# UMEssen/Body-and-Organ-Analysis

Hardware: AMD Instinct MI355X
Metric: CT volumes/sec (512^3 @1.5 mm, total+bca) on MI355X (higher is better)
Workload: dtype f16

## Files before the change

### body-and-organ-analysis_amd/csrc/conv_ns.hip

```cpp
#include <stdlib.h>

#include "conv.h"

#include "conv_ws_dev.h"

#define NS_SW_ROW 24
#define NS_SW_YODD 5
#define NS_SW_ZODD 10
__host__ __device__ constexpr int ns_sw_yp(int y) { return (y & 1) * NS_SW_YODD + (y >> 1); }
__host__ __device__ constexpr int ns_sw_zp(int z) { return (z & 1) * NS_SW_ZODD + (z >> 1); }
__host__ __device__ constexpr int ns_sw_slots() { return 9 * 9 * NS_SW_ROW; }
__host__ __device__ constexpr int ns_sw_plane_bytes() { return (ns_sw_slots() + 8) * 16 + 64; }

template <bool X3, bool SS, bool EDGE>
__device__ __forceinline__ void ns_commit_items_sw(const ConvArgs& p, const ChunkRegs& rg, unsigned char* d0, const int (&off)[WS_MAXV], int plane,
                                                   int nv, unsigned slope2) {
    if (EDGE)
        asm volatile("; commit sw: edge tile");
    else
        asm volatile("; commit sw: interior tile");
#pragma unroll
    for (int j = 0; j < WS_MAXV; ++j) {
        if (j < nv) {
            if constexpr (X3) {
                float y[4] = {__uint_as_float(rg.d[j].x), __uint_as_float(rg.d[j].y), __uint_as_float(rg.d[j].z), __uint_as_float(rg.d[j].w)};
                if (SS) {
#pragma unroll
                    for (int i = 0; i < 4; ++i) {
                        const float f = __builtin_fmaf(y[i], __uint_as_float(rg.ssw[2 * i]), __uint_as_float(rg.ssw[2 * i + 1]));
                        y[i] = f > 0.f ? f : f * p.slope;
                    }
                }
                uint2 hi, lo;
                x3_split4(y, hi, lo);
                if (EDGE && !((rg.ok >> j) & 1u)) hi = lo = make_uint2(0, 0);
                *(uint2*)(d0 + off[j]) = hi;
                *(uint2*)(d0 + plane + off[j]) = lo;
            } else {
                uint4 o = rg.d[j];
                if (SS) o = norm_act8_pk(o, rg.ssw, slope2);
                if (EDGE && !((rg.ok >> j) & 1u)) o = make_uint4(0, 0, 0, 0);
                *(uint4*)(d0 + off[j]) = o;
            }
        }
    }
}

template <bool X3>
__device__ __forceinline__ void ns_commit_sw(const ConvArgs& p, ChunkRegs& rg, unsigned char* dst_in, const int (&off)[WS_MAXV], int q, int HV,
                                             int plane, int dbg) {
    const int nv = (dbg & 32) ? 0 : (HV + WS_PROD / 2 - 1) / (WS_PROD / 2);
    if (rg.skip_halo) return;
    union {
        unsigned u;
        h2_t v;
    } sl2;
    sl2.v = h2_t{(_Float16)p.slope, (_Float16)p.slope};
    unsigned char* d0 = X3 ? dst_in + (q & 1) * 8 : dst_in + (q & 1) * plane;
    const bool edge = __builtin_amdgcn_ballot_w64(rg.ok != rg.live) != 0;
    if (rg.has_ss) {
        if (edge)
            ns_commit_items_sw<X3, true, true>(p, rg, d0, off, plane, nv, sl2.u);
        else
            ns_commit_items_sw<X3, true, false>(p, rg, d0, off, plane, nv, sl2.u);
    } else {
        if (edge)
            ns_commit_items_sw<X3, false, true>(p, rg, d0, off, plane, nv, sl2.u);
        else
            ns_commit_items_sw<X3, false, false>(p, rg, d0, off, plane, nv, sl2.u);
    }
}

template <int S, int RM, bool X3, int NR>
__device__ __forceinline__ void consume_chunk_x(const unsigned char* b0p, f32x16 (&acc)[RM], f16x8 (&a)[NR][3], f16x8 (&al)[X3 ? NR : 1][3],
                                                const WS_GLOBAL unsigned char* wb, unsigned vcur, unsigned vnext, unsigned gs, unsigned lo_off) {
    constexpr int NB = S * (RM - 1) + 3;
    constexpr int MM = X3 ? 2 : 1;
    f16x8 b[NB];
    auto fetch_a = [&](unsigned vchunk, int g, int slot) {
#pragma unroll
        for (int dx = 0; dx < 3; ++dx) {
            unsigned vo = __umul24((unsigned)(g + 9 * dx), gs) + vchunk;
            asm volatile("" : "+v"(vo));
            a[slot][dx] = *(const WS_GLOBAL f16x8*)(wb + vo);
            if constexpr (X3) {
                unsigned vl = vo + lo_off;
                asm volatile("" : "+v"(vl));
                al[slot][dx] = *(const WS_GLOBAL f16x8*)(wb + vl);
            }
        }
    };
#pragma unroll
    for (int jj = 0; jj < NB; ++jj) b[jj] = *(const f16x8*)(b0p + jj * 9 * NS_SW_ROW * 16);
    __builtin_amdgcn_sched_group_barrier(0x100, NB, 0);
#pragma unroll
    for (int g = 0; g < 9; ++g) {
        const int slot = g % NR;
        if (g + NR - 1 < 9)
            fetch_a(vcur, g + NR - 1, (g + NR - 1) % NR);
        else
            fetch_a(vnext, g + NR - 1 - 9, (g + NR - 1) % NR);
        __builtin_amdgcn_sched_group_barrier(0x020, 3 * MM, 0);
#pragma unroll
        for (int jj = 0; jj < NB; ++jj) {
            int cnt = 0;
#pragma unroll
            for (int dx = 0; dx < 3; ++dx) {
                const int rr = jj - dx;
                if (rr < 0 || rr % S != 0 || rr / S >= RM) continue;
                const int r = rr / S;
                acc[r] = __builtin_amdgcn_mfma_f32_32x32x16_f16(a[slot][dx], b[jj], acc[r], 0, 0, 0);
                if constexpr (X3) acc[r] = __builtin_amdgcn_mfma_f32_32x32x16_f16(al[slot][dx], b[jj], acc[r], 0, 0, 0);
                ++cnt;
            }
            if (cnt == 1)
                __builtin_amdgcn_sched_group_barrier(0x008, 1 * MM, 0);
            else if (cnt == 2)
                __builtin_amdgcn_sched_group_barrier(0x008, 2 * MM, 0);
            else if (cnt == 3)
                __builtin_amdgcn_sched_group_barrier(0x008, 3 * MM, 0);
            if (g + 1 < 9) {
                const int gn = g + 1, dy = gn / 3, dz = gn % 3;
                b[jj] = *(const f16x8*)(b0p + ((jj * 9 + ns_sw_yp(dy)) * NS_SW_ROW + ns_sw_zp(dz)) * 16);
                __builtin_amdgcn_sched_group_barrier(0x100, 1, 0);
            }
        }
    }
}

template <int S, int WN, int RM, bool X3>
__global__ __launch_bounds__(WS_THREADS) void k_conv_ns(ConvArgs p, int dbg_arg, const int* __restrict__ desc, int desc_row) {
    static_assert(S == 2, "k_conv_ns: the halo layout is the stride-2 one");
#ifdef WS_WITH_TRACE
    const int dbg = dbg_arg;
#else
    constexpr int dbg = 0;
    (void)dbg_arg;
#endif
    extern __shared__ __attribute__((aligned(16))) unsigned char smem[];
    const int tid = threadIdx.x;
    const int lane = tid & 63;
    const int wave = __builtin_amdgcn_readfirstlane(tid >> 6);
    const bool producer = wave >= 4;
    const int l31 = lane & 31;
    const int kh = lane >> 5;
    const int HV = p.h0 * p.h1 * p.h2;
    const int plane = ns_sw_plane_bytes();
    const int ncc = (p.C0 + p.C1) / 16;
    const int buf_bytes = 2 * plane;
    unsigned char* bufs = smem;

    const int* __restrict__ drow = desc + (size_t)blockIdx.x * desc_row * 8;
    const int my_tiles = drow[0];
    const int my_chunks = my_tiles * ncc;
    for (int i = tid; i < p.Cout; i += WS_THREADS) ((float*)(smem + 2 * buf_bytes))[i] = p.bias[i];
    const int tr_blk = WS_TRACING ? (int)p.trace[WS_TRACE_SLOTS - 5] : -1;

    if (producer) {
        const int q = tid - 256;
        const ProdConst pc = prod_const(p, q, HV);
        int ldso[WS_MAXV];
#pragma unroll
        for (int j = 0; j < WS_MAXV; ++j) {
            const int v = (q >> 1) + (WS_PROD / 2) * j;
            const int hz = v % 17, t = v / 17;
            const int hy = t % 9, hx = t / 9;
            ldso[j] = (v < HV ? (hx * 9 + ns_sw_yp(hy)) * NS_SW_ROW + ns_sw_zp(hz) : ns_sw_slots()) * 16;
        }
        TileDesc pd;
        pd.flags = pd.vo = pd.ibase = 0;
        TileCoord& ptc = pd.tc;
        int pk = 0;
        ptc.n = ptc.cy = ptc.ox0 = ptc.oy0 = ptc.oz0 = ptc.sp = 0;
        ProdItems items;
#pragma unroll
        for (int j = 0; j < WS_MAXV; ++j) items.gi[j] = 0;
        items.ok = 0;
        constexpr bool PF2 = RM == 4;
        ChunkRegs rgA, rgB;
        auto clear_regs = [&](ChunkRegs& rg) {
#pragma unroll
            for (int j = 0; j < WS_MAXV; ++j) rg.d[j] = make_uint4(0, 0, 0, 0);
#pragma unroll
            for (int j = 0; j < 8; ++j) rg.ssw[j] = 0;
            rg.ok = rg.live = 0;
            rg.has_ss = 0;
            rg.skip_halo = 0;
            rg.cc = rg.cy = 0;
        };
        clear_regs(rgA);
        clear_regs(rgB);
        int pcc = 0;
        int ptr_n = 0;
#define NS_PSTAMP(code)                                                                                                          \
    do {                                                                                                                         \
        if (WS_TRACING && (int)blockIdx.x == tr_blk && wave == 4 && lane == 0 && ptr_n < WS_TRACE_SLOTS / 2 - 8) {                                  \
            p.trace[WS_TRACE_SLOTS / 2 + ptr_n] = ((unsigned long long)(code) << 56) | (__builtin_readcyclecounter() & 0x00ffffffffffffffull); \
            ++ptr_n;                                                                                                             \
        }                                                                                                                        \
    } while (0)
        const bool live = !(dbg & 2);
        auto setup_next = [&]() {
            pd = load_desc(drow, ++pk);
            prod_setup_desc(p, pd, pc, items);
            NS_PSTAMP(8);
        };
        auto issue = [&](ChunkRegs& rg) {
            prod_issue(p, ptc, items, pc.in_halo, pcc, false, q, dbg, rg);
            if (++pcc == ncc) pcc = 0;
            NS_PSTAMP(3);
        };
        auto commit = [&](ChunkRegs& rg, unsigned char* dst) {
            if (WS_TRACING) {
                asm volatile("s_waitcnt vmcnt(0)" ::: "memory");
                NS_PSTAMP(7);
            }
            ns_commit_sw<X3>(p, rg, dst, ldso, q, HV, plane, dbg);
            NS_PSTAMP(2);
        };
        if (live && my_chunks > 0) {
            pd = load_desc(drow, 0);
            prod_setup_desc(p, pd, pc, items);
            prod_issue(p, ptc, items, pc.in_halo, 0, false, q, dbg, rgA);
            if (++pcc == ncc) pcc = 0;
        }
        if constexpr (PF2) {
            auto interval = [&](int g, ChunkRegs& cur, ChunkRegs& nxt) {
                if (live && g + 1 < my_chunks) {
                    NS_PSTAMP(1);
                    if (g + 2 < my_chunks) {
                        if (pcc == 0) setup_next();
                        issue(nxt);
                    }
                    commit(cur, bufs + ((g + 1) & 1) * buf_bytes);
                }
                __syncthreads();
            };
            for (int g = -1; g < my_chunks; g += 2) {
                interval(g, rgA, rgB);
                if (g + 1 < my_chunks) interval(g + 1, rgB, rgA);
            }
        } else {
            for (int g = -1; g < my_chunks; ++g) {
                if (live && g + 1 < my_chunks) {
                    NS_PSTAMP(1);
                    const bool do_issue = g + 2 < my_chunks;
                    if (do_issue && pcc == 0) setup_next();
                    commit(rgA, bufs + ((g + 1) & 1) * buf_bytes);
                    if (do_issue) issue(rgA);
                }
                __syncthreads();
            }
        }
        return;
    }

    if (!(dbg & 1024)) __builtin_amdgcn_s_setprio(3);
    int tr_n = 0;
#define NS_STAMP(code)                                                                                                   \
    do {                                                                                                                 \
        if (WS_TRACING && (int)blockIdx.x == tr_blk && wave == 0 && lane == 0 && tr_n < WS_TRACE_SLOTS / 2) {                              \
            p.trace[tr_n] = ((unsigned long long)(code) << 56) | (__builtin_readcyclecounter() & 0x00ffffffffffffffull); \
            ++tr_n;                                                                                                      \
        }                                                                                                                \
    } while (0)
    const int cw = wave & 3;
    const int wn = cw % WN, wm = cw / WN;
    const int ly = l31 >> 3, lz = l31 & 7;
    const int nchunks_out = p.Cout / 32;
    const int hoff = (((2 * (wm * RM)) * 9 + ly) * NS_SW_ROW + lz) * 16 + kh * plane;
    const int srel0 = ly * p.Wo + lz;
    const size_t out_vox = (size_t)p.Do * p.Ho * p.Wo;
    const int nslots = p.nslots;
    int slot = 0;
    float st_s[16], st_q[16];
#pragma unroll
    for (int i = 0; i < 16; ++i) st_s[i] = st_q[i] = 0.f;
    int st_n = -1, st_ch = 0;
    auto flush_stats = [&]() {
        if (st_n < 0) return;
#define NS_HALVE(M, HALF)                                                                                \
    {                                                                                                    \
        const bool up = (l31 & (M)) != 0;                                                                \
        _Pragma("unroll") for (int i = 0; i < (HALF); ++i) {                                             \
            const float ks = up ? st_s[i + (HALF)] : st_s[i], gs_ = up ? st_s[i] : st_s[i + (HALF)];     \
            const float kq = up ? st_q[i + (HALF)] : st_q[i], gq_ = up ? st_q[i] : st_q[i + (HALF)];     \
            st_s[i] = ks + __shfl_xor(gs_, (M));                                                         \
            st_q[i] = kq + __shfl_xor(gq_, (M));                                                         \
        }                                                                                                \
    }
        NS_HALVE(1, 8)
        NS_HALVE(2, 4)
        NS_HALVE(4, 2)
        NS_HALVE(8, 1)
#undef NS_HALVE
        st_s[0] += __shfl_xor(st_s[0], 16);
        st_q[0] += __shfl_xor(st_q[0], 16);
        if (l31 < 16) {
            const int i = ((l31 & 1) << 3) | ((l31 & 2) << 1) | ((l31 & 4) >> 1) | ((l31 & 8) >> 3);
            const int row = st_ch * 32 + 8 * (i >> 2) + 4 * kh + (i & 3);
            float* pp = p.partials + (((size_t)st_n * p.Cout + row) * 2) * nslots + slot;
            pp[0] = st_s[0];
            pp[nslots] = st_q[0];
        }
#pragma unroll
        for (int i = 0; i < 16; ++i) st_s[i] = st_q[i] = 0.f;
    };

    f32x16 acc[RM];
    auto epilogue = [&](const TileCoord& tc, int ch, int dfl, int dvo) {
        st_n = tc.n;
        st_ch = ch;
        const int cout0 = ch * 32;
        const bool full = (dfl & WS_DF_FULL) != 0;
        const size_t ovox = (size_t)(unsigned)dvo;
        const size_t obase = ((size_t)tc.n * p.Cout + cout0) * out_vox + ovox * 16;
        const unsigned olane = ((unsigned)kh * (unsigned)out_vox + (unsigned)srel0) * 32u;
#pragma unroll
        for (int r = 0; r < RM; ++r) {
            const int mx = wm * RM + r;
            const int mrel = mx * p.Ho * p.Wo;
            bool ok = true;
            if (!full) ok = tc.ox0 + mx < p.Do && tc.oy0 + ly < p.Ho && tc.oz0 + lz < p.Wo;
            const float dm = ok ? 1.f : 0.f;
            float v[16];
#pragma unroll
            for (int i = 0; i < 16; ++i) v[i] = X3 ? acc[r][i] * p.winv : acc[r][i];
#pragma unroll
            for (int i = 0; i < 8; ++i) {
                f2_t vm = f2_t{v[2 * i], v[2 * i + 1]};
                if (!full) vm = vm * f2_t{dm, dm};
                f2_t s2 = f2_t{st_s[2 * i], st_s[2 * i + 1]}, q2 = f2_t{st_q[2 * i], st_q[2 * i + 1]};
                s2 = s2 + vm;
                q2 = __builtin_elementwise_fma(vm, vm, q2);
                st_s[2 * i] = s2.x; st_s[2 * i + 1] = s2.y;
                st_q[2 * i] = q2.x; st_q[2 * i + 1] = q2.y;
            }
            if constexpr (X3) {
                if (ok && !(dbg & 4)) {
                    const size_t doff = ((size_t)tc.n * p.Cout + cout0) * out_vox * 4 + (ovox + (size_t)mrel) * 32;
                    const unsigned dlo = __builtin_amdgcn_readfirstlane((unsigned)doff), dhi = __builtin_amdgcn_readfirstlane((unsigned)(doff >> 32));
                    WS_GLOBAL unsigned char* dst = sgpr_ptr((const unsigned char*)p.out + (((size_t)dhi << 32) | dlo));
#pragma unroll
                    for (int gq = 0; gq < 4; ++gq) {
                        unsigned ol = ((unsigned)srel0 * 32u + (unsigned)kh * 16u) + (unsigned)gq * ((unsigned)out_vox * 32u);
                        asm volatile("" : "+v"(ol));
                        __builtin_nontemporal_store(f32x4_t{v[gq * 4 + 0], v[gq * 4 + 1], v[gq * 4 + 2], v[gq * 4 + 3]}, (WS_GLOBAL f32x4_t*)(dst + ol));
                    }
                }
                continue;
            }
            __builtin_amdgcn_sched_barrier(0);
            unsigned w[8];
#pragma unroll
            for (int pr = 0; pr < 2; ++pr) {
                float lo4[4], hi4[4];
#pragma unroll
                for (int e = 0; e < 4; ++e) {
                    const auto sw = __builtin_amdgcn_permlane32_swap(__float_as_uint(v[pr * 4 + e]), __float_as_uint(v[(pr + 2) * 4 + e]), false, false);
                    lo4[e] = __uint_as_float(sw[0]);
                    hi4[e] = __uint_as_float(sw[1]);
                }
                w[pr * 4 + 0] = cvt_pk_h2(lo4[0], lo4[1]);
                w[pr * 4 + 1] = cvt_pk_h2(lo4[2], lo4[3]);
                w[pr * 4 + 2] = cvt_pk_h2(hi4[0], hi4[1]);
                w[pr * 4 + 3] = cvt_pk_h2(hi4[2], hi4[3]);
            }
            if (ok && !(dbg & 4)) {
                WS_GLOBAL unsigned char* dst = sgpr_ptr(p.out + (obase + (size_t)mrel * 16));
                unsigned ol = olane;
                asm volatile("" : "+v"(ol));
                __builtin_nontemporal_store(u32x4_t{w[0], w[1], w[2], w[3]}, (WS_GLOBAL u32x4_t*)(dst + ol));
                __builtin_nontemporal_store(u32x4_t{w[4], w[5], w[6], w[7]}, (WS_GLOBAL u32x4_t*)(dst + ol + 16));
            }
        }
    };

    const unsigned gs = 32u * (unsigned)p.Cout;
    const unsigned voff = X3 ? (unsigned)l31 * 16u : ((unsigned)kh * (unsigned)p.Cout + (unsigned)l31) * 16u;
    const unsigned lo_off = (unsigned)p.Cout * 16u;
    auto woff = [&](int cc, int ch) -> unsigned { return voff + (unsigned)cc * 27u * gs + (unsigned)ch * 512u; };
    constexpr int NR = (RM == 2 && !X3) ? 9 : 3;
    f16x8 a[NR][3];
    f16x8 al[X3 ? NR : 1][3];
#pragma unroll
    for (int i = 0; i < NR; ++i)
#pragma unroll
        for (int j = 0; j < 3; ++j)
#pragma unroll
            for (int e = 0; e < 8; ++e) {
                a[i][j][e] = (_Float16)0.f;
                if (X3 || i == 0) al[X3 ? i : 0][j][e] = (_Float16)0.f;
            }
    auto prime = [&](unsigned vchunk) {
        const WS_GLOBAL unsigned char* wb = sgpr_ptr(p.wpk);
#pragma unroll
        for (int g = 0; g < NR - 1; ++g)
#pragma unroll
            for (int dx = 0; dx < 3; ++dx) {
                unsigned vo = __umul24((unsigned)(g + 9 * dx), gs) + vchunk;
                asm volatile("" : "+v"(vo));
                a[g][dx] = *(const WS_GLOBAL f16x8*)(wb + vo);
                if constexpr (X3) {
                    unsigned vl = vo + lo_off;
                    asm volatile("" : "+v"(vl));
                    al[g][dx] = *(const WS_GLOBAL f16x8*)(wb + vl);
                }
            }
    };

    TileDesc cd;
    cd.flags = cd.vo = cd.ibase = 0;
    cd.tc.n = cd.tc.cy = cd.tc.ox0 = cd.tc.oy0 = cd.tc.oz0 = cd.tc.sp = 0;
    bool ring_valid = false;
    TileCoord done_tc = cd.tc;
    int done_ch = 0, done_fl = 0, done_vo = 0;
    bool done_active = false;
    __syncthreads();
    for (int k = 0; k < my_tiles + 1; ++k) {
        const bool more = k < my_tiles;
        bool new_run = true;
        NS_STAMP(1);
        if (more) {
            cd = load_desc(drow, k);
            new_run = (cd.flags & WS_DF_NEWRUN) != 0;
        }
        const bool have_next = k + 1 < my_tiles;
        const TileCoord& tc = cd.tc;
        const int ch = tc.cy * WN + wn;
        if (k > 0 && done_active && !(dbg & 8)) epilogue(done_tc, done_ch, done_fl, done_vo);
        if (k > 0 && (!more || new_run || tc.n != st_n || ch != st_ch)) {
            flush_stats();
            st_n = -1;
        }
        if (!more) break;
        if (new_run) slot = (int)((unsigned)cd.flags >> 16) * 4 + cw;
        const bool active = ch < nchunks_out;
        int ch_next = have_next ? drow[(size_t)(k + 2) * 8 + 1] * WN + wn : ch;
        const bool next_active = have_next && ch_next < nchunks_out;
        if (ch_next >= nchunks_out) ch_next = nchunks_out - 1;
        if (active) {
            const float* lb = (const float*)(smem + 2 * buf_bytes) + ch * 32 + 4 * kh;
#pragma unroll
            for (int gq = 0; gq < 4; ++gq) {
                const f32x4_t bv = *(const f32x4_t*)(lb + 8 * gq);
#pragma unroll
                for (int r = 0; r < RM; ++r) {
                    acc[r][gq * 4 + 0] = X3 ? bv[0] * p.wscale : bv[0]; acc[r][gq * 4 + 1] = X3 ? bv[1] * p.wscale : bv[1];
                    acc[r][gq * 4 + 2] = X3 ? bv[2] * p.wscale : bv[2]; acc[r][gq * 4 + 3] = X3 ? bv[3] * p.wscale : bv[3];
                }
            }
            if (!ring_valid) prime(woff(0, ch));
        }
        NS_STAMP(2);
        for (int cc = 0; cc < ncc; ++cc) {
            const int g = k * ncc + cc;
            if (active) {
                const unsigned char* cur = bufs + (g & 1) * buf_bytes;
                int ho = hoff;
                asm volatile("" : "+v"(ho));
                const WS_GLOBAL unsigned char* wb = sgpr_ptr(p.wpk);
                const unsigned vcur = woff(cc, ch);
                const unsigned vnext = cc + 1 < ncc ? woff(cc + 1, ch) : woff(0, ch_next);
                consume_chunk_x<S, RM, X3, NR>(cur + ho, acc, a, al, wb, vcur, vnext, gs, lo_off);
            }
            NS_STAMP(3);
            __syncthreads();
            NS_STAMP(4);
        }
        ring_valid = active && next_active;
        done_tc.n = __builtin_amdgcn_readfirstlane(tc.n);
        done_tc.cy = __builtin_amdgcn_readfirstlane(tc.cy);
        done_tc.sp = __builtin_amdgcn_readfirstlane(tc.sp);
        done_tc.ox0 = __builtin_amdgcn_readfirstlane(tc.ox0);
        done_tc.oy0 = __builtin_amdgcn_readfirstlane(tc.oy0);
        done_tc.oz0 = __builtin_amdgcn_readfirstlane(tc.oz0);
        done_ch = __builtin_amdgcn_readfirstlane(ch);
        done_fl = __builtin_amdgcn_readfirstlane(cd.flags);
        done_vo = __builtin_amdgcn_readfirstlane(cd.vo);
        done_active = active;
    }
}

const int* ws_run_table(boa_ctx* ctx, const ConvArgs& a, int tiles_per_sample, int vw);
const int* ws_desc_table(boa_ctx* ctx, const ConvArgs& a, int tiles_per_sample, int grid, int* row_out);
int conv_ws_vw(int tiles_per_sample, int cu_count);

bool conv_ns_applicable(const ConvGeom& g) {
    const bool k333 = g.k[0] == 3 && g.k[1] == 3 && g.k[2] == 3;
    const bool s2 = g.s[0] == 2 && g.s[1] == 2 && g.s[2] == 2;
    if (!k333 || g.Cout % 32 != 0) return false;
    return s2 && g.Cout >= 64 && g.Do >= 8 && g.Ho >= 8 && g.Wo >= 8;
}

static int ns_wn(int Cout) { return Cout >= 128 ? 4 : 2; }
int conv_ns_wn(int Cout) { return ns_wn(Cout); }

void conv_ns_tile(const ConvGeom& g, ConvTile* t) {
    t->variant = 2;
    t->xs = 0;
    t->R = 4;
    t->w[0] = 1; t->w[1] = 4; t->w[2] = 8;
    t->b[0] = 4; t->b[1] = 1; t->b[2] = 1;
    const int ext[3] = {4, 4, 8};
    const int dims[3] = {g.Do, g.Ho, g.Wo};
    for (int d = 0; d < 3; ++d) {
        t->h[d] = (ext[d] - 1) * g.s[d] + 3;
        t->tiles[d] = (dims[d] + ext[d] - 1) / ext[d];
    }
    t->lds_bytes = 4 * (size_t)ns_sw_plane_bytes() + (size_t)g.Cout * sizeof(float);
}

int conv_ns_ncy(int Cout) { return (Cout / 32 + ns_wn(Cout) - 1) / ns_wn(Cout); }

template <int S, int WN, int RM, bool X3 = false>
static void launch_ns(boa_ctx* ctx, const ConvArgs& a, const ConvTile& t, int grid, const int* desc, int desc_row) {
    static bool once = (hipFuncSetAttribute((const void*)k_conv_ns<S, WN, RM, X3>, hipFuncAttributeMaxDynamicSharedMemorySize, 160 * 1024), true);
    (void)once;
    hipLaunchKernelGGL((k_conv_ns<S, WN, RM, X3>), dim3(grid), dim3(WS_THREADS), t.lds_bytes, ctx->stream, a,
                       getenv("BOA_WS_DBG") ? atoi(getenv("BOA_WS_DBG")) : 0, desc, desc_row);
}

int launch_conv_ns(boa_ctx* ctx, const ConvArgs& a_in, const ConvTile& t, double flops, double bytes, bool x3) {
    ConvArgs a = a_in;
    a.ncy = conv_ns_ncy(a.Cout);
    const int total = t.tiles[0] * t.tiles[1] * t.tiles[2] * a.ncy;
    const int vw = conv_ws_vw(total, ctx->cu_count);
    const int grid = (int)std::min<long long>((long long)vw * a.N, ctx->cu_count);
    BOA_REQUIRE((double)a.Di * a.Hi * a.Wi <= 16777216.0, "conv_ns: more than 2^24 input voxels per sample (24-bit offset multiply)");
    BOA_REQUIRE((double)a.Di * a.Hi * a.Wi * std::max(a.C0, a.C1) * 2.0 < 4294967296.0,
                "conv_ns: one sample of the input exceeds 4 GiB (32-bit voxel offsets)");
    BOA_REQUIRE(2 * t.h[0] * t.h[1] * t.h[2] <= WS_PROD * WS_MAXV, "conv_ns: halo too large");
#ifdef WS_WITH_TRACE
    static const bool want_trace = getenv("BOA_WS_TRACE") != nullptr;
#else
    static const bool want_trace = false;
#endif
    a.trace = nullptr;
    if (want_trace) {
        hipMalloc(&a.trace, WS_TRACE_SLOTS * 8);
        hipMemsetAsync(a.trace, 0, WS_TRACE_SLOTS * 8, ctx->stream);
        const unsigned long long blk = (unsigned long long)std::min(std::max(atoi(getenv("BOA_WS_TRACE")), 0), grid - 1);
        hipMemcpyAsync(a.trace + WS_TRACE_SLOTS - 5, &blk, 8, hipMemcpyHostToDevice, ctx->stream);
    }
    a.nslots = 4 * vw;
    a.vw = vw;
    a.vstep_n = grid / vw;
    a.vstep_j = grid % vw;
    a.cy_fast = 0;
    a.runs = ws_run_table(ctx, a, total, vw);
    BOA_REQUIRE(a.runs != nullptr, "conv_ns: could not allocate the run table");
    int desc_row = 0;
    const int* desc = ws_desc_table(ctx, a, total, grid, &desc_row);
    BOA_REQUIRE(desc != nullptr, "conv_ns: could not allocate the tile descriptor table");
    KernelTimer tm(ctx, BOA_K_CONV_MFMA, flops, bytes);
    ctx->counters[x3 ? BOA_CNT_CONV_X3 : BOA_CNT_CONV_WS]++;
    BOA_REQUIRE(a.s0 == 2, "conv_ns: instantiated for stride 2 only");
    if (x3) {
        if (ns_wn(a.Cout) == 2)
            launch_ns<2, 2, 2, true>(ctx, a, t, grid, desc, desc_row);
        else
            launch_ns<2, 4, 4, true>(ctx, a, t, grid, desc, desc_row);
    } else if (ns_wn(a.Cout) == 2)
        launch_ns<2, 2, 2>(ctx, a, t, grid, desc, desc_row);
    else
        launch_ns<2, 4, 4>(ctx, a, t, grid, desc, desc_row);
    tm.stop();
    if (want_trace && a.trace) {
        static unsigned long long host[WS_TRACE_SLOTS];
        hipStreamSynchronize(ctx->stream);
        hipMemcpy(host, a.trace, sizeof(host), hipMemcpyDeviceToHost);
        hipFree(a.trace);
        fprintf(stderr, "[ns-trace] Cin=%d Cout=%d in=%d s=%d:", a.C0 + a.C1, a.Cout, a.Di, a.s0);
        for (int i = 1; i < 80 && host[i]; ++i)
            fprintf(stderr, " %d:%llu", (int)(host[i] >> 56), (host[i] & 0x00ffffffffffffffull) - (host[i - 1] & 0x00ffffffffffffffull));
        fprintf(stderr, "\n[ns-trace] producer:");
        const unsigned long long* hp = host + WS_TRACE_SLOTS / 2;
        for (int i = 41; i < 110 && hp[i]; ++i)
            fprintf(stderr, " %d:%llu", (int)(hp[i] >> 56), (hp[i] & 0x00ffffffffffffffull) - (hp[i - 1] & 0x00ffffffffffffffull));
        fprintf(stderr, "\n");
    }
    BOA_HIP_TRY(hipGetLastError());
    return BOA_OK;
}
```

### body-and-organ-analysis_amd/csrc/conv_ws_dev.h

```cpp
#pragma once
#include "conv.h"
#define WS_THREADS 512
#define WS_PROD (WS_THREADS - 256)
#define WS_WB ((27 * 64 + WS_PROD - 1) / WS_PROD)
#define WS_TRACE_SLOTS 4096
#ifndef WS_WITH_TRACE
#define WS_STAMP(code) do { } while (0)
#define WS_TRACING false
#else
#define WS_TRACING (p.trace != nullptr)
#define WS_STAMP(code)                                                                          \
    do {                                                                                        \
        if (p.trace && (int)blockIdx.x == tr_blk && lane == 0 && ((wave & 3) == 0) && tr_n < WS_TRACE_SLOTS / 2) { \
            p.trace[(producer ? WS_TRACE_SLOTS / 2 : 0) + tr_n] = ((unsigned long long)(code) << 56) | (__builtin_readcyclecounter() & 0x00ffffffffffffffull); \
            ++tr_n;                                                                             \
        }                                                                                       \
    } while (0)
#endif

__device__ __forceinline__ int ws_plane_bytes(int HV) { return ((HV + WS_PROD / 2 - 1) / (WS_PROD / 2)) * (WS_PROD / 2) * 16 + 64; }

struct TileCoord {
    int n, cy, ox0, oy0, oz0;
    int sp;
};

__device__ __forceinline__ TileCoord decode_tile(const ConvArgs& p, int t) {
    TileCoord c;
    const int nsp = p.t0 * p.t1 * p.t2;
    const int ncy = p.ncy;
    if (p.cy_fast) {
        c.cy = t % ncy;
        const int r = t / ncy;
        c.sp = r % nsp;
        c.n = r / nsp;
    } else {
        c.sp = t % nsp;
        const int r = t / nsp;
        c.cy = r % ncy;
        c.n = r / ncy;
    }
    int bt = c.sp;
    const int tx = bt % p.t0;
    bt /= p.t0;
    const int tz = bt % p.t2;
    const int ty = bt / p.t2;
    c.ox0 = tx * p.b0 * p.w0;
    c.oy0 = ty * p.b1 * p.w1;
    c.oz0 = tz * p.b2 * p.w2;
    return c;
}

__device__ __forceinline__ void next_tile(const ConvArgs& p, TileCoord& c) {
    const int e0 = p.b0 * p.w0, e1 = p.b1 * p.w1, e2 = p.b2 * p.w2;
    const int ncy = p.ncy;
    if (p.cy_fast) {
        if (++c.cy < ncy) return;
        c.cy = 0;
    }
    ++c.sp;
    c.ox0 += e0;
    if (c.ox0 >= p.t0 * e0) {
        c.ox0 = 0;
        c.oz0 += e2;
        if (c.oz0 >= p.t2 * e2) {
            c.oz0 = 0;
            c.oy0 += e1;
            if (c.oy0 >= p.t1 * e1) {
                c.oy0 = 0;
                c.sp = 0;
                if (p.cy_fast) {
                    ++c.n;
                } else if (++c.cy >= ncy) {
                    c.cy = 0;
                    ++c.n;
                }
            }
        }
    }
}

struct TileSeq {
    int n, j;
    int left;
    TileCoord tc;
};

__device__ __forceinline__ void seq_run(const ConvArgs& p, TileSeq& s) {
    const int* r = p.runs + s.j * 8;
    s.left = r[0];
    s.tc.n = s.n;
    s.tc.cy = r[1];
    s.tc.sp = r[2];
    s.tc.ox0 = r[3];
    s.tc.oy0 = r[4];
    s.tc.oz0 = r[5];
}

__device__ __forceinline__ void seq_first_of(const ConvArgs& p, TileSeq& s, int blk) {
    s.n = blk / p.vw;
    s.j = blk - s.n * p.vw;
    seq_run(p, s);
}
__device__ __forceinline__ void seq_first(const ConvArgs& p, TileSeq& s) { seq_first_of(p, s, (int)blockIdx.x); }

__device__ __forceinline__ bool seq_next(const ConvArgs& p, TileSeq& s) {
    if (--s.left > 0) {
        next_tile(p, s.tc);
        return false;
    }
    s.n += p.vstep_n;
    s.j += p.vstep_j;
    if (s.j >= p.vw) {
        s.j -= p.vw;
        ++s.n;
    }
    seq_run(p, s);
    return true;
}

#define WS_DF_NEWRUN 1
#define WS_DF_FULL 2
#define WS_DF_REUSE 4

struct TileDesc {
    TileCoord tc;
    int flags, vo, ibase;
};

__device__ __forceinline__ TileDesc make_desc(const ConvArgs& p, const TileSeq& s, bool new_run) {
    TileDesc d;
    d.tc = s.tc;
    const TileCoord& tc = s.tc;
    int fl = new_run ? WS_DF_NEWRUN : 0;
    if (tc.ox0 + p.b0 * p.w0 <= p.Do && tc.oy0 + p.b1 * p.w1 <= p.Ho && tc.oz0 + p.b2 * p.w2 <= p.Wo) fl |= WS_DF_FULL;
    if (p.cy_fast && tc.cy != 0 && !new_run) fl |= WS_DF_REUSE;
    const int ix0 = tc.ox0 * p.s0 - p.p0, iy0 = tc.oy0 * p.s1 - p.p1, iz0 = tc.oz0 * p.s2 - p.p2;
    if (ix0 >= 0 && iy0 >= 0 && iz0 >= 0 && ix0 + p.h0 <= p.Di && iy0 + p.h1 <= p.Hi && iz0 + p.h2 <= p.Wi) {
    } else if (ix0 >= -1 && iy0 >= -1 && iz0 >= -1 && ix0 + p.h0 <= p.Di + 1 && iy0 + p.h1 <= p.Hi + 1 && iz0 + p.h2 <= p.Wi + 1) {
        fl |= 1 << 4;
        fl |= (ix0 < 0 ? 1 : 0) << 8 | (ix0 + p.h0 > p.Di ? 1 : 0) << 9 | (iy0 < 0 ? 1 : 0) << 10 | (iy0 + p.h1 > p.Hi ? 1 : 0) << 11 |
              (iz0 < 0 ? 1 : 0) << 12 | (iz0 + p.h2 > p.Wi ? 1 : 0) << 13;
    } else {
        fl |= 2 << 4;
    }
    fl |= s.j << 16;
    d.flags = fl;
    d.vo = (tc.ox0 * p.Ho + tc.oy0) * p.Wo + tc.oz0;
    d.ibase = (ix0 * p.Hi + iy0) * p.Wi + iz0;
    return d;
}

__device__ __forceinline__ TileDesc load_desc(const int* __restrict__ row, int k) {
    const int4 a = *(const int4*)(row + (size_t)(k + 1) * 8), b = *(const int4*)(row + (size_t)(k + 1) * 8 + 4);
    TileDesc d;
#define WS_U(x) __builtin_amdgcn_readfirstlane(x)
    d.tc.n = WS_U(a.x); d.tc.cy = WS_U(a.y); d.tc.ox0 = WS_U(a.z); d.tc.oy0 = WS_U(a.w); d.tc.oz0 = WS_U(b.x); d.tc.sp = 0;
    d.flags = WS_U(b.y); d.vo = WS_U(b.z); d.ibase = WS_U(b.w);
#undef WS_U
    return d;
}

#define WS_MAXV (2 * 1536 / WS_PROD)

struct ProdConst {
    int rel[WS_MAXV];
    int hc[WS_MAXV];
    unsigned in_halo;
    unsigned face[6];
};

__device__ __forceinline__ ProdConst prod_const(const ConvArgs& p, int q, int HV) {
    ProdConst k;
    k.in_halo = 0;
#pragma unroll
    for (int f = 0; f < 6; ++f) k.face[f] = 0;
#pragma unroll
    for (int j = 0; j < WS_MAXV; ++j) {
        const int v = (q >> 1) + (WS_PROD / 2) * j;
        const int hx = v / p.xs, rem = v - hx * p.xs;
        const int hz = rem % p.h2, hy = rem / p.h2;
        const bool in = v < HV && hy < p.h1;
        k.rel[j] = in ? (hx * p.Hi + hy) * p.Wi + hz : 0;
        k.hc[j] = in ? (hx | (hy << 10) | (hz << 20)) : 0;
        const unsigned bit = in ? (1u << j) : 0u;
        k.in_halo |= bit;
        k.face[0] |= hx == 0 ? bit : 0u;
        k.face[1] |= hx == p.h0 - 1 ? bit : 0u;
        k.face[2] |= hy == 0 ? bit : 0u;
        k.face[3] |= hy == p.h1 - 1 ? bit : 0u;
        k.face[4] |= hz == 0 ? bit : 0u;
        k.face[5] |= hz == p.h2 - 1 ? bit : 0u;
    }
    return k;
}

struct ProdItems {
    int gi[WS_MAXV];
    unsigned ok;
};

__device__ __forceinline__ void prod_setup(const ConvArgs& p, const TileCoord& tc, const ProdConst& k, ProdItems& it) {
    const int ix0 = tc.ox0 * p.s0 - p.p0, iy0 = tc.oy0 * p.s1 - p.p1, iz0 = tc.oz0 * p.s2 - p.p2;
    const int base = (ix0 * p.Hi + iy0) * p.Wi + iz0;
    const bool interior = ix0 >= 0 && iy0 >= 0 && iz0 >= 0 && ix0 + p.h0 <= p.Di && iy0 + p.h1 <= p.Hi && iz0 + p.h2 <= p.Wi;
    if (interior) {
        it.ok = k.in_halo;
#pragma unroll
        for (int j = 0; j < WS_MAXV; ++j) it.gi[j] = base + k.rel[j];
    } else if (ix0 >= -1 && iy0 >= -1 && iz0 >= -1 && ix0 + p.h0 <= p.Di + 1 && iy0 + p.h1 <= p.Hi + 1 && iz0 + p.h2 <= p.Wi + 1) {
        unsigned out = 0;
        out |= ix0 < 0 ? k.face[0] : 0u;
        out |= ix0 + p.h0 > p.Di ? k.face[1] : 0u;
        out |= iy0 < 0 ? k.face[2] : 0u;
        out |= iy0 + p.h1 > p.Hi ? k.face[3] : 0u;
        out |= iz0 < 0 ? k.face[4] : 0u;
        out |= iz0 + p.h2 > p.Wi ? k.face[5] : 0u;
        const unsigned okm = k.in_halo & ~out;
        it.ok = okm;
#pragma unroll
        for (int j = 0; j < WS_MAXV; ++j) it.gi[j] = ((okm >> j) & 1u) ? base + k.rel[j] : 0;
    } else {
        unsigned okm = 0;
#pragma unroll
        for (int j = 0; j < WS_MAXV; ++j) {
            const unsigned ix = (unsigned)(ix0 + (k.hc[j] & 1023)), iy = (unsigned)(iy0 + ((k.hc[j] >> 10) & 1023)),
                           iz = (unsigned)(iz0 + (k.hc[j] >> 20));
            const unsigned ok = (unsigned)(ix < (unsigned)p.Di) & (unsigned)(iy < (unsigned)p.Hi) & (unsigned)(iz < (unsigned)p.Wi) &
                                ((k.in_halo >> j) & 1u);
            it.gi[j] = ok ? base + k.rel[j] : 0;
            okm |= ok << j;
        }
        it.ok = okm;
    }
}

__device__ __forceinline__ void prod_setup_desc(const ConvArgs& p, const TileDesc& d, const ProdConst& k, ProdItems& it) {
    const int cls = (d.flags >> 4) & 3;
    const int base = d.ibase;
    if (cls == 0) {
        it.ok = k.in_halo;
#pragma unroll
        for (int j = 0; j < WS_MAXV; ++j) it.gi[j] = base + k.rel[j];
    } else if (cls == 1) {
        unsigned out = 0;
#pragma unroll
        for (int f = 0; f < 6; ++f) out |= (d.flags >> (8 + f)) & 1 ? k.face[f] : 0u;
        const unsigned okm = k.in_halo & ~out;
        it.ok = okm;
#pragma unroll
        for (int j = 0; j < WS_MAXV; ++j) it.gi[j] = ((okm >> j) & 1u) ? base + k.rel[j] : 0;
    } else {
        prod_setup(p, d.tc, k, it);
    }
}

typedef unsigned u32x4_t __attribute__((ext_vector_type(4)));
typedef float f32x4_t __attribute__((ext_vector_type(4)));
#define WS_GLOBAL __attribute__((address_space(1)))
__device__ __forceinline__ WS_GLOBAL unsigned char* sgpr_ptr(const void* p) {
    const size_t v = (size_t)p;
    const unsigned lo = __builtin_amdgcn_readfirstlane((unsigned)v), hi = __builtin_amdgcn_readfirstlane((unsigned)(v >> 32));
    WS_GLOBAL unsigned char* g = (WS_GLOBAL unsigned char*)(((size_t)hi << 32) | lo);
    asm volatile("" : "+s"(g));
    return g;
}

#define OPAQUE4(a) "+v"((a).x), "+v"((a).y), "+v"((a).z), "+v"((a).w)

typedef unsigned int u32x4_t __attribute__((ext_vector_type(4)));
__device__ __forceinline__ void touch128(uint4& a) {
    u32x4_t t = {a.x, a.y, a.z, a.w};
    asm volatile("" : "+v"(t));
    a = make_uint4(t.x, t.y, t.z, t.w);
}

typedef _Float16 h2_t __attribute__((ext_vector_type(2)));

typedef float f2_t __attribute__((ext_vector_type(2)));
__device__ __forceinline__ unsigned cvt_pk_h2(float a, float b) {
    union {
        h2_t v;
        unsigned u;
    } c;
    c.v = __builtin_convertvector(f2_t{a, b}, h2_t);
    return c.u;
}

__device__ __forceinline__ uint4 norm_act8_pk(uint4 raw, const unsigned* w , unsigned slope2) {
    union {
        uint4 u;
        h2_t v[4];
    } x;
    union {
        unsigned u;
        h2_t v;
    } s, t, sl;
    x.u = raw;
    sl.u = slope2;
    h2_t y[4], z[4];
#pragma unroll
    for (int i = 0; i < 4; ++i) {
        s.u = w[2 * i];
        t.u = w[2 * i + 1];
        y[i] = __builtin_elementwise_fma(x.v[i], s.v, t.v);
    }
#pragma unroll
    for (int i = 0; i < 4; ++i) z[i] = y[i] * sl.v;
#pragma unroll
    for (int i = 0; i < 4; ++i) x.v[i] = __builtin_elementwise_max(y[i], z[i]);
    return x.u;
}

struct ChunkRegs {
    uint4 d[WS_MAXV];
    unsigned ssw[8];
    unsigned ok;
    unsigned live;
    int has_ss;
    int skip_halo;
    int cc, cy;
};

__device__ __forceinline__ void prod_issue(const ConvArgs& p, const TileCoord& tc, const ProdItems& it, unsigned live, int cc,
                                           bool skip_halo, int q, int dbg, ChunkRegs& rg) {
    int cg = cc * 16;
    const size_t in_vox = (size_t)p.Di * p.Hi * p.Wi;
    const __half* base;
    const unsigned* ss;
    int C;
    if (cg < p.C0) {
        base = p.src0 + ((size_t)tc.n * p.C0 + cg) * in_vox;
        ss = p.ss16_0 ? p.ss16_0 + ((size_t)tc.n * p.C0 + cg) : nullptr;
        C = p.C0;
    } else {
        cg -= p.C0;
        base = p.src1 + ((size_t)tc.n * p.C1 + cg) * in_vox;
        ss = p.ss16_1 ? p.ss16_1 + ((size_t)tc.n * p.C1 + cg) : nullptr;
        C = p.C1;
    }
    (void)C;
    if (dbg & 64) ss = nullptr;
    rg.skip_halo = skip_halo;
    if (skip_halo) return;
    rg.ok = it.ok;
    rg.live = live;
    rg.has_ss = ss != nullptr;
    const unsigned cb2 = 32u;
    const unsigned char* sbase = (const unsigned char*)base;
    const unsigned lane_off = (unsigned)(q & 1) * 16u;
    const int nrounds = (p.h0 * p.xs + WS_PROD / 2 - 1) / (WS_PROD / 2);
#pragma unroll
    for (int j = 0; j < WS_MAXV; ++j) {
        if (j < nrounds && !(dbg & 128))
        rg.d[j] = *(const uint4*)(sbase + (__umul24((unsigned)it.gi[j], cb2) + lane_off));
    }
    if (ss) {
        unsigned so = (unsigned)(q & 1) * 32u;
        asm volatile("" : "+v"(so));
        const uint4 s0 = *(const uint4*)((const unsigned char*)ss + so);
        const uint4 s1 = *(const uint4*)((const unsigned char*)ss + so + 16);
        rg.ssw[0] = s0.x; rg.ssw[1] = s0.y; rg.ssw[2] = s0.z; rg.ssw[3] = s0.w;
        rg.ssw[4] = s1.x; rg.ssw[5] = s1.y; rg.ssw[6] = s1.z; rg.ssw[7] = s1.w;
    }
}

__device__ __forceinline__ void dma_weights(const ConvArgs& p, int cc, int cy, unsigned char* dst_w, int q, int taps) {
    const int nw = taps * 64;
    const __half* wsrc = p.wpk + ((size_t)cc * taps * 2) * p.Cout * 8 + (size_t)cy * 32 * 8;
    const unsigned lds0 = (unsigned)(size_t)dst_w + (unsigned)((q >> 6) * 64) * 16u;
#pragma unroll
    for (int b = 0; b < WS_WB; ++b) {
        const int i = q + b * WS_PROD;
        if (i < nw) {
            const unsigned voff = ((unsigned)(i >> 5) * (unsigned)p.Cout + (unsigned)(i & 31)) * 16u;
            const unsigned m0v = __builtin_amdgcn_readfirstlane(lds0 + (unsigned)(b * WS_PROD) * 16u);
            unsigned keep;
            asm volatile("s_mov_b32 %0, m0\n\ts_mov_b32 m0, %3\n\ts_nop 0\n\tglobal_load_lds_dwordx4 %1, %2\n\ts_mov_b32 m0, %0"
                         : "=&s"(keep)
                         : "v"(voff), "s"(wsrc), "s"(m0v)
                         : "memory");
        }
    }
}

template <bool SS, bool EDGE>
__device__ __forceinline__ void commit_items(const ChunkRegs& rg, unsigned char* d0, int nv, unsigned slope2) {
    if (EDGE)
        asm volatile("; commit: edge tile");
    else
        asm volatile("; commit: interior tile");
#pragma unroll
    for (int j = 0; j < WS_MAXV; ++j) {
        if (j < nv) {
            uint4 o = rg.d[j];
            if (SS) o = norm_act8_pk(o, rg.ssw, slope2);
            if (EDGE && !((rg.ok >> j) & 1u)) o = make_uint4(0, 0, 0, 0);
            *(uint4*)(d0 + j * (WS_PROD / 2 * 16)) = o;
        }
    }
}

__device__ __forceinline__ void prod_commit(const ConvArgs& p, ChunkRegs& rg, unsigned char* dst_in, int q, int HV, int plane,
                                            int dbg) {
    const int nv = (dbg & 32) ? 0 : (HV + WS_PROD / 2 - 1) / (WS_PROD / 2);
    if (rg.skip_halo) return;
    union {
        unsigned u;
        h2_t v;
    } sl2;
    sl2.v = h2_t{(_Float16)p.slope, (_Float16)p.slope};
    unsigned char* d0 = dst_in + (q & 1) * plane + (q >> 1) * 16;
    const bool edge = __builtin_amdgcn_ballot_w64(rg.ok != rg.live) != 0;
    if (rg.has_ss) {
        if (edge)
            commit_items<true, true>(rg, d0, nv, sl2.u);
        else
            commit_items<true, false>(rg, d0, nv, sl2.u);
    } else {
        if (edge)
            commit_items<false, true>(rg, d0, nv, sl2.u);
        else
            commit_items<false, false>(rg, d0, nv, sl2.u);
    }
}

__device__ __forceinline__ void x3_split4(const float (&y)[4], uint2& hi, uint2& lo) {
    union {
        h2_t v;
        unsigned u;
    } h01, h23;
    h01.v = __builtin_convertvector(f2_t{y[0], y[1]}, h2_t);
    h23.v = __builtin_convertvector(f2_t{y[2], y[3]}, h2_t);
    const float r0 = y[0] - (float)h01.v[0], r1 = y[1] - (float)h01.v[1], r2 = y[2] - (float)h23.v[0], r3 = y[3] - (float)h23.v[1];
    hi = make_uint2(h01.u, h23.u);
    lo = make_uint2(cvt_pk_h2(r0, r1), cvt_pk_h2(r2, r3));
}

template <bool SS, bool EDGE>
__device__ __forceinline__ void commit_items_x3(const ChunkRegs& rg, unsigned char* d0, int plane, int nv, float slope) {
    if (EDGE)
        asm volatile("; commit x3: edge tile");
    else
        asm volatile("; commit x3: interior tile");
#pragma unroll
    for (int j = 0; j < WS_MAXV; ++j) {
        if (j < nv) {
            float y[4] = {__uint_as_float(rg.d[j].x), __uint_as_float(rg.d[j].y), __uint_as_float(rg.d[j].z), __uint_as_float(rg.d[j].w)};
            if (SS) {
#pragma unroll
                for (int i = 0; i < 4; ++i) {
                    const float f = __builtin_fmaf(y[i], __uint_as_float(rg.ssw[2 * i]), __uint_as_float(rg.ssw[2 * i + 1]));
                    y[i] = f > 0.f ? f : f * slope;
                }
            }
            uint2 hi, lo;
            x3_split4(y, hi, lo);
            if (EDGE && !((rg.ok >> j) & 1u)) hi = lo = make_uint2(0, 0);
            *(uint2*)(d0 + j * (WS_PROD / 2 * 16)) = hi;
            *(uint2*)(d0 + plane + j * (WS_PROD / 2 * 16)) = lo;
        }
    }
}

__device__ __forceinline__ void prod_commit_x3(const ConvArgs& p, ChunkRegs& rg, unsigned char* dst_in, int q, int HV, int plane, int dbg) {
    const int nv = (dbg & 32) ? 0 : (HV + WS_PROD / 2 - 1) / (WS_PROD / 2);
    if (rg.skip_halo) return;
    unsigned char* d0 = dst_in + (q >> 1) * 16 + (q & 1) * 8;
    const bool edge = __builtin_amdgcn_ballot_w64(rg.ok != rg.live) != 0;
    if (rg.has_ss) {
        if (edge)
            commit_items_x3<true, true>(rg, d0, plane, nv, p.slope);
        else
            commit_items_x3<true, false>(rg, d0, plane, nv, p.slope);
    } else {
        if (edge)
            commit_items_x3<false, true>(rg, d0, plane, nv, p.slope);
        else
            commit_items_x3<false, false>(rg, d0, plane, nv, p.slope);
    }
}
```

Baseline: 0.5955.

## Roll producer halo loads into per-item commit loop with single register set

Restructures the producer waves of the conv_ns kernel so that each halo item is committed to shared memory and then immediately reloaded with the next chunk's data, using one register set instead of double-buffered A/B registers. The producer is specialised for the fixed 9x9x17 halo, with compile-time item counts and a new inline descriptor setup. The intent is to cut producer register pressure and interleave global loads with LDS stores more tightly. In exchange, the kernel now requires that exact halo shape, and load latency is hidden by only one item of lead.

Result: faster. 0.6024 (median of 6 runs) (+1.2%).

```diff
diff --git a/body-and-organ-analysis_amd/csrc/conv_ns.hip b/body-and-organ-analysis_amd/csrc/conv_ns.hip
--- a/body-and-organ-analysis_amd/csrc/conv_ns.hip
+++ b/body-and-organ-analysis_amd/csrc/conv_ns.hip
@@ -12,63 +12,127 @@
 __host__ __device__ constexpr int ns_sw_slots() { return 9 * 9 * NS_SW_ROW; }
 __host__ __device__ constexpr int ns_sw_plane_bytes() { return (ns_sw_slots() + 8) * 16 + 64; }
 
+#define NS_HV (9 * 9 * 17)
+#define NS_ITEMS ((NS_HV + WS_PROD / 2 - 1) / (WS_PROD / 2))
+static_assert(NS_ITEMS <= WS_MAXV, "k_conv_ns: halo items per producer lane");
+
+__device__ __forceinline__ unsigned ns_setup_desc(const ConvArgs& p, const TileDesc& d, const ProdConst& k, int (&gi)[NS_ITEMS]) {
+    const int cls = (d.flags >> 4) & 3;
+    const int base = d.ibase;
+    unsigned okm;
+    if (cls == 0) {
+        okm = k.in_halo;
+#pragma unroll
+        for (int j = 0; j < NS_ITEMS; ++j) gi[j] = base + k.rel[j];
+    } else if (cls == 1) {
+        unsigned out = 0;
+#pragma unroll
+        for (int f = 0; f < 6; ++f) out |= (d.flags >> (8 + f)) & 1 ? k.face[f] : 0u;
+        okm = k.in_halo & ~out;
+#pragma unroll
+        for (int j = 0; j < NS_ITEMS; ++j) gi[j] = ((okm >> j) & 1u) ? base + k.rel[j] : 0;
+    } else {
+        const int ix0 = d.tc.ox0 * p.s0 - p.p0, iy0 = d.tc.oy0 * p.s1 - p.p1, iz0 = d.tc.oz0 * p.s2 - p.p2;
+        okm = 0;
+#pragma unroll
+        for (int j = 0; j < NS_ITEMS; ++j) {
+            const unsigned ix = (unsigned)(ix0 + (k.hc[j] & 1023)), iy = (unsigned)(iy0 + ((k.hc[j] >> 10) & 1023)),
+                           iz = (unsigned)(iz0 + (k.hc[j] >> 20));
+            const unsigned ok = (unsigned)(ix < (unsigned)p.Di) & (unsigned)(iy < (unsigned)p.Hi) & (unsigned)(iz < (unsigned)p.Wi) &
+                                ((k.in_halo >> j) & 1u);
+            gi[j] = ok ? base + k.rel[j] : 0;
+            okm |= ok << j;
+        }
+    }
+    return okm;
+}
+
+struct NsRegs {
+    u32x4_t d[NS_ITEMS];
+    u32x4_t s0, s1;
+    unsigned ok, live;
+    int has_ss;
+};
+
 template <bool X3, bool SS, bool EDGE>
-__device__ __forceinline__ void ns_commit_items_sw(const ConvArgs& p, const ChunkRegs& rg, unsigned char* d0, const int (&off)[WS_MAXV], int plane,
-                                                   int nv, unsigned slope2) {
+__device__ __forceinline__ void ns_commit_item_sw(const ConvArgs& p, const u32x4_t& d, const unsigned (&w)[8], bool ok, unsigned char* d0, int off,
+                                                  int plane, unsigned slope2) {
+    if constexpr (X3) {
+        float y[4] = {__uint_as_float(d.x), __uint_as_float(d.y), __uint_as_float(d.z), __uint_as_float(d.w)};
+        if (SS) {
+#pragma unroll
+            for (int i = 0; i < 4; ++i) {
+                const float f = __builtin_fmaf(y[i], __uint_as_float(w[2 * i]), __uint_as_float(w[2 * i + 1]));
+                y[i] = f > 0.f ? f : f * p.slope;
+            }
+        }
+        uint2 hi, lo;
+        x3_split4(y, hi, lo);
+        if (EDGE && !ok) hi = lo = make_uint2(0, 0);
+        *(uint2*)(d0 + off) = hi;
+        *(uint2*)(d0 + plane + off) = lo;
+    } else {
+        uint4 o = make_uint4(d.x, d.y, d.z, d.w);
+        if (SS) o = norm_act8_pk(o, w, slope2);
+        if (EDGE && !ok) o = make_uint4(0, 0, 0, 0);
+        *(uint4*)(d0 + off) = o;
+    }
+}
+
+template <bool X3, bool SS, bool EDGE, bool ISSUE>
+__device__ __forceinline__ void ns_roll_items_sw(const ConvArgs& p, NsRegs& rg, const unsigned (&w_in)[8], unsigned ok, unsigned char* d0,
+                                                 const int (&off)[WS_MAXV], int plane, unsigned slope2, const unsigned char* nbase,
+                                                 const int (&gi)[NS_ITEMS], int q, int dbg) {
+    unsigned w[8];
+#pragma unroll
+    for (int i = 0; i < 8; ++i) w[i] = w_in[i];
+#define NS_ROLL_MARK(text) \
+    asm volatile(text : "+v"(w[0]), "+v"(w[1]), "+v"(w[2]), "+v"(w[3]), "+v"(w[4]), "+v"(w[5]), "+v"(w[6]), "+v"(w[7]), "+v"(slope2))
     if (EDGE)
-        asm volatile("; commit sw: edge tile");
+        NS_ROLL_MARK("; roll sw: edge tile");
     else
-        asm volatile("; commit sw: interior tile");
-#pragma unroll
-    for (int j = 0; j < WS_MAXV; ++j) {
-        if (j < nv) {
-            if constexpr (X3) {
-                float y[4] = {__uint_as_float(rg.d[j].x), __uint_as_float(rg.d[j].y), __uint_as_float(rg.d[j].z), __uint_as_float(rg.d[j].w)};
-                if (SS) {
-#pragma unroll
-                    for (int i = 0; i < 4; ++i) {
-                        const float f = __builtin_fmaf(y[i], __uint_as_float(rg.ssw[2 * i]), __uint_as_float(rg.ssw[2 * i + 1]));
-                        y[i] = f > 0.f ? f : f * p.slope;
-                    }
-                }
-                uint2 hi, lo;
-                x3_split4(y, hi, lo);
-                if (EDGE && !((rg.ok >> j) & 1u)) hi = lo = make_uint2(0, 0);
-                *(uint2*)(d0 + off[j]) = hi;
-                *(uint2*)(d0 + plane + off[j]) = lo;
-            } else {
-                uint4 o = rg.d[j];
-                if (SS) o = norm_act8_pk(o, rg.ssw, slope2);
-                if (EDGE && !((rg.ok >> j) & 1u)) o = make_uint4(0, 0, 0, 0);
-                *(uint4*)(d0 + off[j]) = o;
-            }
-        }
-    }
-}
-
-template <bool X3>
-__device__ __forceinline__ void ns_commit_sw(const ConvArgs& p, ChunkRegs& rg, unsigned char* dst_in, const int (&off)[WS_MAXV], int q, int HV,
-                                             int plane, int dbg) {
-    const int nv = (dbg & 32) ? 0 : (HV + WS_PROD / 2 - 1) / (WS_PROD / 2);
-    if (rg.skip_halo) return;
+        NS_ROLL_MARK("; roll sw: interior tile");
+#undef NS_ROLL_MARK
+#pragma unroll
+    for (int j = 0; j < NS_ITEMS; ++j) {
+        if (!(dbg & 32)) ns_commit_item_sw<X3, SS, EDGE>(p, rg.d[j], w, (ok >> j) & 1u, d0, off[j], plane, slope2);
+        __builtin_amdgcn_sched_barrier(0);
+        if (ISSUE && !(dbg & 128)) rg.d[j] = prod_load_item<u32x4_t>(nbase, gi[j], q);
+        __builtin_amdgcn_sched_barrier(0);
+    }
+}
+
+__device__ __forceinline__ void ns_issue_head(const ChunkSrc& src, unsigned ok, unsigned live, int q, NsRegs& rg) {
+    rg.ok = ok;
+    rg.live = live;
+    rg.has_ss = src.ss != nullptr;
+    if (src.ss) prod_load_ss(src.ss, q, rg.s0, rg.s1);
+    __builtin_amdgcn_sched_barrier(0);
+}
+
+template <bool X3, bool ISSUE>
+__device__ __forceinline__ void ns_roll_sw(const ConvArgs& p, NsRegs& rg, unsigned char* dst_in, const int (&off)[WS_MAXV], int q, int plane,
+                                           const ChunkSrc& src, const int (&gi)[NS_ITEMS], unsigned iok, unsigned live, int dbg) {
+    unsigned w[8] = {rg.s0.x, rg.s0.y, rg.s0.z, rg.s0.w, rg.s1.x, rg.s1.y, rg.s1.z, rg.s1.w};
+    asm volatile("" : "+v"(w[0]), "+v"(w[1]), "+v"(w[2]), "+v"(w[3]), "+v"(w[4]), "+v"(w[5]), "+v"(w[6]), "+v"(w[7]));
+    const unsigned ok = rg.ok;
+    const bool has_ss = rg.has_ss != 0;
+    const bool edge = __builtin_amdgcn_ballot_w64(rg.ok != rg.live) != 0;
+    int form = __builtin_amdgcn_readfirstlane((has_ss ? 2 : 0) | (edge ? 1 : 0));
+    if (ISSUE) ns_issue_head(src, iok, live, q, rg);
     union {
         unsigned u;
         h2_t v;
     } sl2;
     sl2.v = h2_t{(_Float16)p.slope, (_Float16)p.slope};
     unsigned char* d0 = X3 ? dst_in + (q & 1) * 8 : dst_in + (q & 1) * plane;
-    const bool edge = __builtin_amdgcn_ballot_w64(rg.ok != rg.live) != 0;
-    if (rg.has_ss) {
-        if (edge)
-            ns_commit_items_sw<X3, true, true>(p, rg, d0, off, plane, nv, sl2.u);
-        else
-            ns_commit_items_sw<X3, true, false>(p, rg, d0, off, plane, nv, sl2.u);
-    } else {
-        if (edge)
-            ns_commit_items_sw<X3, false, true>(p, rg, d0, off, plane, nv, sl2.u);
-        else
-            ns_commit_items_sw<X3, false, false>(p, rg, d0, off, plane, nv, sl2.u);
-    }
+    if (form == 3) ns_roll_items_sw<X3, true, true, ISSUE>(p, rg, w, ok, d0, off, plane, sl2.u, src.base, gi, q, dbg);
+    asm volatile("" : "+s"(form));
+    if (form == 2) ns_roll_items_sw<X3, true, false, ISSUE>(p, rg, w, ok, d0, off, plane, sl2.u, src.base, gi, q, dbg);
+    asm volatile("" : "+s"(form));
+    if (form == 1) ns_roll_items_sw<X3, false, true, ISSUE>(p, rg, w, ok, d0, off, plane, sl2.u, src.base, gi, q, dbg);
+    asm volatile("" : "+s"(form));
+    if (form == 0) ns_roll_items_sw<X3, false, false, ISSUE>(p, rg, w, ok, d0, off, plane, sl2.u, src.base, gi, q, dbg);
 }
 
 template <int S, int RM, bool X3, int NR>
@@ -158,7 +222,7 @@
 
     if (producer) {
         const int q = tid - 256;
-        const ProdConst pc = prod_const(p, q, HV);
+        ProdConst pc = prod_const(p, q, HV);
         int ldso[WS_MAXV];
 #pragma unroll
         for (int j = 0; j < WS_MAXV; ++j) {
@@ -172,24 +236,16 @@
         TileCoord& ptc = pd.tc;
         int pk = 0;
         ptc.n = ptc.cy = ptc.ox0 = ptc.oy0 = ptc.oz0 = ptc.sp = 0;
-        ProdItems items;
-#pragma unroll
-        for (int j = 0; j < WS_MAXV; ++j) items.gi[j] = 0;
-        items.ok = 0;
-        constexpr bool PF2 = RM == 4;
-        ChunkRegs rgA, rgB;
-        auto clear_regs = [&](ChunkRegs& rg) {
-#pragma unroll
-            for (int j = 0; j < WS_MAXV; ++j) rg.d[j] = make_uint4(0, 0, 0, 0);
-#pragma unroll
-            for (int j = 0; j < 8; ++j) rg.ssw[j] = 0;
-            rg.ok = rg.live = 0;
-            rg.has_ss = 0;
-            rg.skip_halo = 0;
-            rg.cc = rg.cy = 0;
-        };
-        clear_regs(rgA);
-        clear_regs(rgB);
+        int gi[NS_ITEMS];
+        unsigned iok = 0;
+#pragma unroll
+        for (int j = 0; j < NS_ITEMS; ++j) gi[j] = 0;
+        NsRegs rg;
+#pragma unroll
+        for (int j = 0; j < NS_ITEMS; ++j) rg.d[j] = u32x4_t{0, 0, 0, 0};
+        rg.s0 = rg.s1 = u32x4_t{0, 0, 0, 0};
+        rg.ok = rg.live = 0;
+        rg.has_ss = 0;
         int pcc = 0;
         int ptr_n = 0;
 #define NS_PSTAMP(code)                                                                                                          \
@@ -200,58 +256,44 @@
         }                                                                                                                        \
     } while (0)
         const bool live = !(dbg & 2);
-        auto setup_next = [&]() {
-            pd = load_desc(drow, ++pk);
-            prod_setup_desc(p, pd, pc, items);
-            NS_PSTAMP(8);
-        };
-        auto issue = [&](ChunkRegs& rg) {
-            prod_issue(p, ptc, items, pc.in_halo, pcc, false, q, dbg, rg);
-            if (++pcc == ncc) pcc = 0;
-            NS_PSTAMP(3);
-        };
-        auto commit = [&](ChunkRegs& rg, unsigned char* dst) {
-            if (WS_TRACING) {
-                asm volatile("s_waitcnt vmcnt(0)" ::: "memory");
-                NS_PSTAMP(7);
-            }
-            ns_commit_sw<X3>(p, rg, dst, ldso, q, HV, plane, dbg);
-            NS_PSTAMP(2);
-        };
         if (live && my_chunks > 0) {
             pd = load_desc(drow, 0);
-            prod_setup_desc(p, pd, pc, items);
-            prod_issue(p, ptc, items, pc.in_halo, 0, false, q, dbg, rgA);
+            iok = ns_setup_desc(p, pd, pc, gi);
+            const ChunkSrc src = prod_chunk_src(p, ptc.n, 0, dbg);
+            ns_issue_head(src, iok, pc.in_halo, q, rg);
+#pragma unroll
+            for (int j = 0; j < NS_ITEMS; ++j)
+                if (!(dbg & 128)) rg.d[j] = prod_load_item<u32x4_t>(src.base, gi[j], q);
             if (++pcc == ncc) pcc = 0;
         }
-        if constexpr (PF2) {
-            auto interval = [&](int g, ChunkRegs& cur, ChunkRegs& nxt) {
-                if (live && g + 1 < my_chunks) {
-                    NS_PSTAMP(1);
-                    if (g + 2 < my_chunks) {
-                        if (pcc == 0) setup_next();
-                        issue(nxt);
-                    }
-                    commit(cur, bufs + ((g + 1) & 1) * buf_bytes);
-                }
-                __syncthreads();
-            };
-            for (int g = -1; g < my_chunks; g += 2) {
-                interval(g, rgA, rgB);
-                if (g + 1 < my_chunks) interval(g + 1, rgB, rgA);
-            }
-        } else {
-            for (int g = -1; g < my_chunks; ++g) {
-                if (live && g + 1 < my_chunks) {
-                    NS_PSTAMP(1);
-                    const bool do_issue = g + 2 < my_chunks;
-                    if (do_issue && pcc == 0) setup_next();
-                    commit(rgA, bufs + ((g + 1) & 1) * buf_bytes);
-                    if (do_issue) issue(rgA);
-                }
-                __syncthreads();
-            }
-        }
+        for (int g = -1; live && g + 2 < my_chunks; ++g) {
+            NS_PSTAMP(1);
+            if (pcc == 0) {
+                pd = load_desc(drow, ++pk);
+#pragma unroll
+                for (int j = 0; j < WS_MAXV; ++j) asm volatile("" : "+v"(pc.hc[j]));
+                asm volatile("" : "+v"(pc.in_halo));
+                iok = ns_setup_desc(p, pd, pc, gi);
+                NS_PSTAMP(8);
+            }
+            const ChunkSrc src = prod_chunk_src(p, ptc.n, pcc, dbg);
+            if (++pcc == ncc) pcc = 0;
+            ns_roll_sw<X3, true>(p, rg, bufs + ((g + 1) & 1) * buf_bytes, ldso, q, plane, src, gi, iok, pc.in_halo, dbg);
+            NS_PSTAMP(2);
+            __syncthreads();
+        }
+        if (live && my_chunks > 0) {
+            NS_PSTAMP(1);
+            ChunkSrc none;
+            none.base = nullptr;
+            none.ss = nullptr;
+            ns_roll_sw<X3, false>(p, rg, bufs + ((my_chunks - 1) & 1) * buf_bytes, ldso, q, plane, none, gi, iok, pc.in_halo, dbg);
+            NS_PSTAMP(2);
+            __syncthreads();
+        }
+        if (!live)
+            for (int g = -1; g + 1 < my_chunks; ++g) __syncthreads();
+        __syncthreads();
         return;
     }
 
@@ -530,7 +572,8 @@
     BOA_REQUIRE((double)a.Di * a.Hi * a.Wi <= 16777216.0, "conv_ns: more than 2^24 input voxels per sample (24-bit offset multiply)");
     BOA_REQUIRE((double)a.Di * a.Hi * a.Wi * std::max(a.C0, a.C1) * 2.0 < 4294967296.0,
                 "conv_ns: one sample of the input exceeds 4 GiB (32-bit voxel offsets)");
-    BOA_REQUIRE(2 * t.h[0] * t.h[1] * t.h[2] <= WS_PROD * WS_MAXV, "conv_ns: halo too large");
+    BOA_REQUIRE(t.h[0] == 9 && t.h[1] == 9 && t.h[2] == 17 && a.h0 * a.h1 * a.h2 == NS_HV && a.xs == a.h1 * a.h2,
+                "conv_ns: the producers are unrolled for the 9 x 9 x 17 halo");
 #ifdef WS_WITH_TRACE
     static const bool want_trace = getenv("BOA_WS_TRACE") != nullptr;
 #else
diff --git a/body-and-organ-analysis_amd/csrc/conv_ws_dev.h b/body-and-organ-analysis_amd/csrc/conv_ws_dev.h
--- a/body-and-organ-analysis_amd/csrc/conv_ws_dev.h
+++ b/body-and-organ-analysis_amd/csrc/conv_ws_dev.h
@@ -322,6 +322,40 @@
     int cc, cy;
 };
 
+struct ChunkSrc {
+    const unsigned char* base;
+    const unsigned* ss;
+};
+
+__device__ __forceinline__ ChunkSrc prod_chunk_src(const ConvArgs& p, int n, int cc, int dbg) {
+    int cg = cc * 16;
+    const size_t in_vox = (size_t)p.Di * p.Hi * p.Wi;
+    ChunkSrc s;
+    if (cg < p.C0) {
+        s.base = (const unsigned char*)(p.src0 + ((size_t)n * p.C0 + cg) * in_vox);
+        s.ss = p.ss16_0 ? p.ss16_0 + ((size_t)n * p.C0 + cg) : nullptr;
+    } else {
+        cg -= p.C0;
+        s.base = (const unsigned char*)(p.src1 + ((size_t)n * p.C1 + cg) * in_vox);
+        s.ss = p.ss16_1 ? p.ss16_1 + ((size_t)n * p.C1 + cg) : nullptr;
+    }
+    if (dbg & 64) s.ss = nullptr;
+    return s;
+}
+
+template <typename T>
+__device__ __forceinline__ T prod_load_item(const unsigned char* sbase, int gi, int q) {
+    return *(const T*)(sbase + (__umul24((unsigned)gi, 32u) + (unsigned)(q & 1) * 16u));
+}
+
+template <typename T>
+__device__ __forceinline__ void prod_load_ss(const unsigned* ss, int q, T& s0, T& s1) {
+    unsigned so = (unsigned)(q & 1) * 32u;
+    asm volatile("" : "+v"(so));
+    s0 = *(const T*)((const unsigned char*)ss + so);
+    s1 = *(const T*)((const unsigned char*)ss + so + 16);
+}
+
 __device__ __forceinline__ void prod_issue(const ConvArgs& p, const TileCoord& tc, const ProdItems& it, unsigned live, int cc,
                                            bool skip_halo, int q, int dbg, ChunkRegs& rg) {
     int cg = cc * 16;
```
